# DaanVrancken/HubbardTN

Measured on AMD Instinct MI355X. Metric: DMRG sweep time (s) + GS energy/site, 1-band Hubbard L=64 chi=1024, lower is better.
Workload: dtype c128; 1 GPU; one-band Hubbard chain L=64 U/t=4, half filling, fZ2xSU(2)xU(1), two-site DMRG sweep (2L-3=125 bond updates) at chi=1024 (TensorKit dim units); model=one_band, L=64, chi=1024, krylovdim=30, parallelism=sector-parallel apply x1, backend=hip

## Files before the change

hubbardtn_amd/csrc/htn_svd.hip:

```cpp
#include <algorithm>
#include <utility>
#include <vector>

#include "htn_common.h"

#ifdef HTN_QR_PROF
#define QR_PROF 1
#else
#define QR_PROF 0
#endif
#ifdef HTN_RING_PROF
#define RING_PROF 1
#else
#define RING_PROF 0
#endif
#define JAC_T_1(var) const long long var = wall_clock64()
#define JAC_T_0(var)
#define JAC_ACC_1(arr, slot, a, b) arr[slot] += (b) - (a)
#define JAC_ACC_0(arr, slot, a, b)
#define JAC_PICK_(name, on) name##on
#define JAC_PICK(name, on) JAC_PICK_(name, on)
#define JAC_T(on, var) JAC_PICK(JAC_T_, on)(var)
#define JAC_ACC(on, arr, slot, a, b) JAC_PICK(JAC_ACC_, on)(arr, slot, a, b)

// ... 141 lines not shown
    static bool attr_set[64] = {};
    int dev = 0;
    HIP_TRY(hipGetDevice(&dev));
    std::lock_guard<std::mutex> lk(attr_mu);
    if (dev >= 0 && dev < 64 && !attr_set[dev]) {
        HIP_TRY(hipFuncSetAttribute((const void*)k_jacobi_svd, hipFuncAttributeMaxDynamicSharedMemorySize,
                                    JAC_LDS_ELEMS * (int)sizeof(double2)));
        HIP_TRY(hipFuncSetAttribute((const void*)k_qr_large, hipFuncAttributeMaxDynamicSharedMemorySize,
                                    16 * (64 * JAC_MAXEL + 1) * (int)sizeof(double2)));
        HIP_TRY(hipFuncSetAttribute((const void*)k_jacobi_pairs_gram, hipFuncAttributeMaxDynamicSharedMemorySize,
                                    (16 * (64 * JAC_MAXEL + 1) + JG_GU_ELEMS) * (int)sizeof(double2)));
        HIP_TRY(hipFuncSetAttribute((const void*)k_jacobi_ring, hipFuncAttributeMaxDynamicSharedMemorySize,
                                    2 * RING_PANEL_ELEMS * (int)sizeof(double2)));
        attr_set[dev] = true;
    }
    return 0;
}

static std::vector<int> classify_large(const htn_svd_block* desc_host, int n_blocks, int split) {
    const int large_min = split > 0 ? std::min(split, JAC_LDS_ELEMS) : JAC_LDS_ELEMS;
    std::vector<int> large;
    if (desc_host)
        for (int b = 0; b < n_blocks; ++b) {
            const htn_svd_block& D = desc_host[b];
            if (!(D.flags & HTN_SVD_QRCP) || D.n < 2) continue;
            if ((int64_t)jac_padded_rows(D.m) * D.n > large_min) large.push_back(b);
        }
    return large;
}

struct JacCoreBufs {
    int *d_ids, *d_slot, *d_perm;
    double* d_zero;
    unsigned long long* d_ratio;
    int *d_done, *d_sw;
    unsigned* d_qsync;
    JacPairItem* d_items;
    JacPairItem* h_items;
    int *h_ids, *h_slot;
    volatile int *h_active, *h_rank, *h_ring_sw;
    int *d_active, *d_rank, *d_ring_sw;
};
static int carve_core_scratch(JacScratch& js, int nl, int n_blocks, int max_sweeps, size_t n_items_max, JacCoreBufs* B) {
    const size_t off_ids = 0, off_slot = off_ids + sizeof(int) * nl, off_perm = off_slot + sizeof(int) * n_blocks;
    const size_t off_zero = off_perm + sizeof(int) * nl * 64 * JAC_MAXEL;
    const size_t off_ratio = (off_zero + sizeof(double) * nl + 7) / 8 * 8, off_done = off_ratio + 16 * nl;
    const size_t off_sw = off_done + sizeof(int) * nl, off_qsync = off_sw + sizeof(int) * nl;
    const size_t off_items = (off_qsync + sizeof(unsigned) * (QR_SYNC_WORDS * (size_t)nl + 8) + 31) / 32 * 32;
    if (js.dev.reserve(off_items + sizeof(JacPairItem) * n_items_max)) return 1;
    if (js.pinned.reserve(sizeof(JacPairItem) * n_items_max + 4 * (size_t)(nl + n_blocks) + 128)) return 1;
    if (js.flags.reserve(sizeof(int) * ((size_t)(max_sweeps + 1) + 2 * (size_t)nl + 16))) return 1;
    char* d = (char*)js.dev.p;
    B->d_ids = (int*)(d + off_ids);
    B->d_slot = (int*)(d + off_slot);
    B->d_perm = (int*)(d + off_perm);
    B->d_zero = (double*)(d + off_zero);
    B->d_ratio = (unsigned long long*)(d + off_ratio);
    B->d_done = (int*)(d + off_done);
    B->d_sw = (int*)(d + off_sw);
    B->d_qsync = (unsigned*)(d + off_qsync);
    B->d_items = (JacPairItem*)(d + off_items);
    char* h = (char*)js.pinned.p;
    B->h_items = (JacPairItem*)h;
    B->h_ids = (int*)(h + sizeof(JacPairItem) * n_items_max);
    B->h_slot = B->h_ids + nl;
    B->h_active = (volatile int*)js.flags.p;
    B->h_rank = B->h_active + (max_sweeps + 1);
    B->h_ring_sw = B->h_rank + nl;
    B->d_active = (int*)js.flags.dev;
    B->d_rank = B->d_active + (max_sweeps + 1);
    B->d_ring_sw = B->d_rank + nl;
    return 0;
}

struct RingPlan {
    std::vector<RingItem> items;
    std::vector<std::pair<int, int>> batches;
    int wgs = 0;
    int64_t mbox_elems = 0;
};
static bool plan_ring(const JacCall& c, int n_xcd, int ring_cap, RingPlan* plan) {
    *plan = RingPlan();
    struct Blk {
        int li, P, w, mp;
    };
    std::vector<Blk> blks;
    for (int li = 0; li < c.nl(); ++li) {
        const htn_svd_block& D = c.desc_host[c.large[li]];
        const int gsx = ring_gs(D.m);
        const int mp = gsx * ring_e(D.m);
        int wcap = std::min(RING_THREADS / gsx, RING_PANEL_ELEMS / mp);
        if (gsx == 16 && wcap > 16 && wcap < 32) wcap = 16;
        if (c.split > 0) wcap = std::min(wcap, 3);
        const int n = std::max(c.n_eff[li], 1);
        const int P = std::max(1, (n + 2 * wcap - 1) / (2 * wcap));
        if (wcap < 1 || P > RING_MAX_P || P > ring_cap) return false;
        blks.push_back({li, P, (n + 2 * P - 1) / (2 * P), mp});
    }
    std::stable_sort(blks.begin(), blks.end(), [](const Blk& a, const Blk& b) { return a.P > b.P; });
    std::vector<char> placed(blks.size(), 0);
    size_t left = blks.size();
    int nx = n_xcd;
    for (const Blk& B : blks)
        if (B.P > ring_cap / nx) nx = 1;
    const int lane_cap = ring_cap / nx;
    while (left) {
        const int first = (int)plan->items.size();
        std::vector<int> lane_used((size_t)nx, 0);
        struct Put {
            int q, x, s0;
        };
        std::vector<Put> puts;
        for (size_t q = 0; q < blks.size(); ++q) {
            if (placed[q]) continue;
            int x = 0;
            for (int y = 1; y < nx; ++y)
                if (lane_used[y] < lane_used[x]) x = y;
            if (lane_used[x] + blks[q].P > lane_cap) continue;
            puts.push_back({(int)q, x, lane_used[x]});
            lane_used[x] += blks[q].P;
            placed[q] = 1;
            --left;
        }
        int depth = 0;
        for (int y = 0; y < nx; ++y) depth = std::max(depth, lane_used[y]);
        const int grid = depth * nx;
        plan->items.resize((size_t)first + grid, RingItem{0, 0, 0, 0, 0, 0, 0});
        for (const Put& pt : puts) {
            const Blk& B = blks[pt.q];
            for (int k = 0; k < B.P; ++k)
                plan->items[(size_t)first + (size_t)(pt.s0 + k) * nx + pt.x] = {B.li, k, B.P, B.w, c.n_eff[B.li], plan->wgs,
                                                                                 plan->mbox_elems};
            plan->mbox_elems += (int64_t)B.P * 4 * B.w * B.mp;
            plan->wgs += B.P;
        }
        plan->batches.push_back({first, grid});
    }
    return true;
}

static int launch_qr_large(const JacCall& c, JacScratch& js, const JacCoreBufs& B, int n_xcd) {
    const int nl = c.nl();
    int max_m0 = 0, min_m0 = 1 << 30, max_n0 = 0;
    for (int b : c.large) {
        max_m0 = std::max(max_m0, (int)c.desc_host[b].pad);
        min_m0 = std::min(min_m0, (int)c.desc_host[b].pad);
        max_n0 = std::max(max_n0, (int)c.desc_host[b].m);
    }
    const size_t qr_panel_elems = (size_t)16 * (((max_m0 + 15) & ~15) + 1);
    const bool coop = ((min_m0 + 15) & ~15) <= 256 && qr_panel_elems * sizeof(double2) + 65536 + 30720 <= 163840;
    const size_t qr_lds = qr_panel_elems * sizeof(double2) + (coop ? 65536 : 0);
    static const bool qr_single = htn_env_flag("HTN_QR_SINGLE");
    static const int env_nw = getenv("HTN_QR_NW") ? atoi(getenv("HTN_QR_NW")) : 0;
    int NW = qr_single ? 1 : ((max_n0 >= 160 || js.xcd_local) ? 4 : 1);
    if (env_nw > 0 && !qr_single) NW = std::min(env_nw, 4);
    const int cus = std::max(1, std::min(js.cu_count > 0 ? js.cu_count : 256, 256));
    const int qnx = (NW > 1 && n_xcd > 1) ? n_xcd : 1;
    const int nl_pad = (nl + qnx - 1) / qnx * qnx;
    NW = std::max(1, std::min(NW, cus / std::max(nl_pad, 1)));
    if (NW > 1 && js.qr_box.reserve((size_t)nl * QR_BOX_BYTES)) return 1;
    const int qgrid_nx = NW > 1 ? qnx : 1;
    hipLaunchKernelGGL(k_qr_large, dim3((NW > 1 ? nl_pad : nl) * NW), dim3(JAC_THREADS), qr_lds, c.st, c.G, c.Vj, c.desc, B.d_ids,
                       B.d_perm, B.d_zero, c.cut2, B.d_rank, NW, (char*)js.qr_box.p, B.d_qsync, nl, qgrid_nx,
                       coop ? (int)qr_panel_elems : 0);
    return 0;
}

static int run_ring(const JacCall& c, JacScratch& js, const JacCoreBufs& B, const RingPlan& plan, int n_xcd, bool two_partner,
                    bool staged_send, int32_t* sweeps_used) {
    const int nl = c.nl(), n_wg = plan.wgs, n_items = (int)plan.items.size();
    const int arrive_off = 2 * n_wg, fail_off = arrive_off + nl * c.max_sweeps, xcc_off = fail_off + 1;
    const int conv_off = (xcc_off + n_wg + 3) & ~3;
    const size_t sync_bytes = ((size_t)conv_off * 4 + (size_t)nl * c.max_sweeps * 16 + 15) & ~(size_t)15;
    if (js.ring_sync.reserve(sync_bytes)) return 1;
    if (js.ring_mbox.reserve(sizeof(double2) * (size_t)std::max<int64_t>(plan.mbox_elems, 1))) return 1;
    if (js.ring_items.reserve(sizeof(RingItem) * n_items) || js.ring_items_h.reserve(sizeof(RingItem) * n_items)) return 1;
    memcpy(js.ring_items_h.p, plan.items.data(), sizeof(RingItem) * n_items);
    for (int li = 0; li < nl; ++li) B.h_ring_sw[li] = 0;
    HIP_TRY(hipMemcpyAsync(js.ring_items.p, js.ring_items_h.p, sizeof(RingItem) * n_items, hipMemcpyHostToDevice, c.st));
    HIP_TRY(hipMemsetAsync(js.ring_sync.p, 0, sync_bytes, c.st));
    RingArgs ra;
    ra.Vj = c.Vj, ra.G = c.G, ra.S = c.S, ra.desc = c.desc, ra.large_ids = B.d_ids;
    ra.perm = B.d_perm, ra.zero2 = B.d_zero, ra.mbox = (double2*)js.ring_mbox.p, ra.sync = (unsigned*)js.ring_sync.p;
    ra.arrive_off = arrive_off, ra.fail_off = fail_off, ra.conv_off = conv_off, ra.max_sweeps = c.max_sweeps, ra.tol = c.tol;
    ra.xcc_off = xcc_off;
    ra.two_partner = two_partner ? 1 : 0;
    ra.staged_send = staged_send ? 1 : 0;
    ra.info = c.info_dev, ra.sweeps_out = B.d_ring_sw;
    for (auto& bt : plan.batches) {
        ra.items = (const RingItem*)js.ring_items.p + bt.first;
        hipLaunchKernelGGL(k_jacobi_ring, dim3((unsigned)bt.second), dim3(RING_THREADS), 2 * RING_PANEL_ELEMS * sizeof(double2),
                           c.st, ra);
    }
    HIP_TRY(hipGetLastError());
    HIP_TRY(hipStreamWaitEvent(c.st, js.ev_join, 0));
    HIP_TRY(htn_stream_spin(c.st));
    int used = 0;
    for (int li = 0; li < nl; ++li) {
        if (B.h_rank[li] < 0) return fail_msg("htn_jacobi_svd_z: a hand-off of the multi-workgroup QR timed out");
        if (B.h_ring_sw[li] <= 0 && c.n_eff[li] >= 2)
            return fail_msg("htn_jacobi_svd_z: a hand-off of the ring Jacobi kernel timed out");
        used = std::max(used, (int)B.h_ring_sw[li] % 1000);
    }
    int all_local = n_xcd > 1 ? 1 : 0;
    for (int li = 0; li < nl; ++li)
        if (c.n_eff[li] >= 2 && B.h_ring_sw[li] < 1000) all_local = 0;
    js.xcd_local = all_local;
    if (sweeps_used) *sweeps_used = used;
    return 0;
}

static int run_pair_visits(const JacCall& c, JacScratch& js, const JacCoreBufs& B, const JacTournament& T, int hint,
                           int32_t* sweeps_used) {
    const int nl = c.nl();
    int max_mp = 0;
    for (int b : c.large) max_mp = std::max(max_mp, jac_padded_rows(c.desc_host[b].m));
    const size_t gram_lds_bytes = (size_t)(16 * (max_mp + 1) + JG_GU_ELEMS) * sizeof(double2);
    const int used = jacobi_sweep_pipeline(c.max_sweeps, hint, js.ev_sweep, B.h_active, c.st, [&](int sweep) {
        for (int r = 0; r < T.n_rounds(); ++r)
            if (T.round_size(r))
                hipLaunchKernelGGL(k_jacobi_pairs_gram, dim3(T.round_size(r)), dim3(256), gram_lds_bytes, c.st, c.Vj, c.desc,
                                   B.d_ids, B.d_items + T.off[r], B.d_zero, B.d_ratio, B.d_done, c.tol, 1);
        hipLaunchKernelGGL(k_jacobi_check, dim3(1), dim3(64), 0, c.st, B.d_ratio, B.d_done, B.d_sw, nl, c.tol, B.d_active + sweep);
    });
    if (used < 0) return 1;
    if (sweeps_used) *sweeps_used = used;
    HIP_TRY(hipStreamWaitEvent(c.st, js.ev_join, 0));
    hipLaunchKernelGGL(k_jacobi_finish, dim3(nl), dim3(JAC_THREADS), 0, c.st, c.G, (const double2*)c.Vj, c.S, c.desc, B.d_ids,
                       B.d_perm, B.d_sw, B.d_done, c.info_dev);
    HIP_TRY(hipGetLastError());
    HIP_TRY(htn_stream_spin(c.st));
    return 0;
}

static int jacobi_svd_core(void* G, void* Vj, double* S, const htn_svd_block* desc, const htn_svd_block* desc_host,
                           int32_t n_blocks, int32_t max_m_host, int32_t max_sweeps, double tol, int32_t* info_dev,
                           const htn_svd_opts* opts, void* stream, const int* skip_dev, const unsigned char* skip_host) {
    if (n_blocks <= 0) return 0;
    if (max_m_host > 64 * JAC_MAXEL) return fail_msg("htn_jacobi_svd_z: block taller than 512 rows");
    const double rank_cut = opts && opts->rank_cut > 0.0 ? opts->rank_cut : 0.0;
    JacCall c = {(double2*)G, (double2*)Vj, S, desc, desc_host, n_blocks, max_sweeps, tol, rank_cut * rank_cut,
                 opts && opts->split_elems > 0 ? opts->split_elems : 0, info_dev, (hipStream_t)stream, {}, {}};
    int32_t* sweeps_used = opts ? opts->sweeps_used : nullptr;
    if (jac_set_kernel_attributes()) return 1;
    c.large = classify_large(desc_host, n_blocks, c.split);
    if (sweeps_used) *sweeps_used = 0;
    if (c.large.empty()) {
        hipLaunchKernelGGL(k_jacobi_svd, dim3(n_blocks), dim3(JAC_THREADS), JAC_LDS_ELEMS * sizeof(double2), c.st, c.G, c.Vj, S,
                           desc, max_sweeps, tol, info_dev, JAC_LDS_ELEMS, skip_dev, c.cut2);
        HIP_TRY(hipGetLastError());
        return 0;
    }
    const int nl = c.nl();
    size_t n_items_max = 0;
    for (int b : c.large) {
        const int nb = (desc_host[b].n + JAC_PANEL - 1) / JAC_PANEL, nbp = nb + (nb & 1);
        n_items_max += (size_t)(nbp - 1) * (nbp / 2) + (nb + 1) / 2;
        c.n_eff.push_back(desc_host[b].n);
    }
    JacScratch* jsp = nullptr;
    JacCoreBufs B;
    if (js_get(c.st, &jsp) || carve_core_scratch(*jsp, nl, n_blocks, max_sweeps, n_items_max, &B)) return 1;
    JacScratch& js = *jsp;
    for (int b = 0; b < n_blocks; ++b) B.h_slot[b] = skip_host && skip_host[b] ? nl : -1;
    for (int li = 0; li < nl; ++li) B.h_slot[c.large[li]] = li;
    for (int li = 0; li < nl; ++li) B.h_ids[li] = c.large[li];
    for (int k = 0; k <= max_sweeps; ++k) B.h_active[k] = 1;
    HIP_TRY(hipMemcpyAsync(B.d_ids, B.h_ids, sizeof(int) * (nl + n_blocks), hipMemcpyHostToDevice, c.st));
    HIP_TRY(hipMemsetAsync(B.d_ratio, 0, 24 * (size_t)nl + sizeof(unsigned) * (QR_SYNC_WORDS * (size_t)nl + 8), c.st));
    static const bool force_pairs = htn_env_flag("HTN_SVD_PAIRS");
    static const bool no_xcd = htn_env_flag("HTN_RING_NO_XCD");
    static const bool ring_staged = htn_env_flag("HTN_RING_STAGED_SEND");
    const bool ring_two_partner = htn_env_flag("HTN_RING_TWO_PARTNER");
    const int n_xcd = (!no_xcd && js.cu_count > 0 && js.cu_count % 8 == 0) ? 8 : 1;
    const int ring_cap = std::max(1, std::min(js.cu_count > 0 ? js.cu_count : 256, 256));
    RingPlan plan;
    JacTournament T;
    bool use_ring = !force_pairs && plan_ring(c, n_xcd, ring_cap, &plan);
    if (c.cut2 <= 0.0 && !use_ring) {
        T = jacobi_tournament(c.n_eff.data(), nl);
        if (upload_tournament(T, B.h_items, B.d_items, c.st)) return 1;
    }
    HIP_TRY(hipEventRecord(js.ev_fork, c.st));
    HIP_TRY(hipStreamWaitEvent(js.aux, js.ev_fork, 0));
    hipLaunchKernelGGL(k_jacobi_svd, dim3(n_blocks), dim3(JAC_THREADS), JAC_LDS_ELEMS * sizeof(double2), js.aux, c.G, c.Vj, S,
                       desc, max_sweeps, tol, info_dev, JAC_LDS_ELEMS, (const int*)B.d_slot, c.cut2);
    HIP_TRY(hipEventRecord(js.ev_join, js.aux));
    if (launch_qr_large(c, js, B, n_xcd)) return 1;
    if (c.cut2 > 0.0) {
        HIP_TRY(hipEventRecord(js.ev_sweep[0], c.st));
        HIP_TRY(htn_event_spin(js.ev_sweep[0]));
        for (int li = 0; li < nl; ++li) c.n_eff[li] = std::min(c.n_eff[li], (int)B.h_rank[li]);
        if (use_ring) use_ring = plan_ring(c, n_xcd, ring_cap, &plan);
        if (!use_ring) {
            T = jacobi_tournament(c.n_eff.data(), nl);
            if (upload_tournament(T, B.h_items, B.d_items, c.st)) return 1;
        }
    }
    if (use_ring) return run_ring(c, js, B, plan, n_xcd, ring_two_partner, ring_staged, sweeps_used);
    return run_pair_visits(c, js, B, T, opts && opts->sweeps_hint > 0 ? opts->sweeps_hint : 0, sweeps_used);
}

static int jacobi_svd_tall(void* G, void* Vj, double* S, const htn_svd_block* desc, const htn_svd_block* desc_host,
                           int32_t n_blocks, int32_t max_m_rest, int32_t max_sweeps, double tol, int32_t* info_dev,
                           const htn_svd_opts* opts, void* stream, const std::vector<int>& tall) {
    const int nt = (int)tall.size();
    hipStream_t st = (hipStream_t)stream;
    JacScratch* jsp = nullptr;
    if (js_get(st, &jsp)) return 1;
    JacScratch& js = *jsp;
    std::vector<int> n_cols(nt);
    for (int li = 0; li < nt; ++li) n_cols[li] = desc_host[tall[li]].n;
// ... 86 lines not shown
```

hubbardtn_amd/csrc/htn_svd_qr.h:

```cpp
#pragma once

template <int GS>
__device__ __forceinline__ int qrcp_mgs(double2* __restrict__ g0, int m0, int n0, int r, const SplitCols X,
                                        int* s_col, double* s_cn2, double* s_piv, int tid, double cut2) {
    const int grp = tid / GS, sub = tid % GS, lane = tid & 63, wave = tid >> 6;
    const int ngroups = JAC_THREADS / GS;
    for (int idx = tid; idx < X.mp * r; idx += JAC_THREADS) X.col(idx / X.mp)[idx % X.mp] = make_double2(0.0, 0.0);
    for (int k = grp; k < n0; k += ngroups) {
        double c = 0.0;
        for (int i = sub; i < m0; i += GS) {
            const double2 x = g0[(int64_t)k * m0 + i];
            c += x.x * x.x + x.y * x.y;
        }
        c = group_sum<GS>(c);
        if (sub == 0) {
            s_cn2[k] = c;
            s_col[k] = k;
        }
    }
    __syncthreads();
    if (wave == 0) {
        double f = 0.0;
        for (int k = lane; k < n0; k += 64) f += s_cn2[k];
        f = wave_sum(f);
        if (lane == 0) s_piv[1] = 1e-30 * f;
    }
    __syncthreads();
    const double zero2 = s_piv[1];
    int rank = 0;
    for (int j = 0; j < r; ++j) {
        if (wave == 0) {
            double best = -1.0, mass = 0.0;
            int bi = j;
            for (int k = j + lane; k < n0; k += 64) {
                mass += s_cn2[k];
                if (s_cn2[k] > best) {
                    best = s_cn2[k];
                    bi = k;
                }
            }
            mass = wave_sum(mass);
#pragma unroll
            for (int off = 32; off > 0; off >>= 1) {
                const double ob = __shfl_xor(best, off, 64);
                const int oi = __shfl_xor(bi, off, 64);
                if (ob > best || (ob == best && oi < bi)) {
                    best = ob;
                    bi = oi;
                }
            }
            if (bi != j)
                for (int jj = lane; jj < j; jj += 64) {
                    double2* xc = X.col(jj);
                    const double2 t = xc[j];
                    xc[j] = xc[bi];
                    xc[bi] = t;
                }
            if (lane == 0) {
                const int t = s_col[j];
                s_col[j] = s_col[bi];
                s_col[bi] = t;
                s_cn2[bi] = s_cn2[j];
                s_cn2[j] = best;
                s_piv[0] = mass <= cut2 ? 0.0 : best;
            }
        }
        __syncthreads();
        if (s_piv[0] <= zero2) break;
        rank = j + 1;
        const double2* __restrict__ p = g0 + (int64_t)s_col[j] * m0;
        for (int k = j + grp; k < n0; k += ngroups) {
            double2 pv[JAC_MAXEL], av[JAC_MAXEL];
            double pp = 0.0, dr = 0.0, di = 0.0;
            double2* __restrict__ a = g0 + (int64_t)s_col[k] * m0;
#pragma unroll
            for (int e = 0; e < JAC_MAXEL; ++e) {
                const int i = sub + GS * e;
                if (i < m0) {
                    pv[e] = p[i];
                    pp += pv[e].x * pv[e].x + pv[e].y * pv[e].y;
                    if (k > j) {
                        av[e] = a[i];
                        dr += pv[e].x * av[e].x + pv[e].y * av[e].y;
                        di += pv[e].x * av[e].y - pv[e].y * av[e].x;
                    }
                }
            }
            pp = group_sum<GS>(pp);
            const double pn = sqrt(pp);
            if (k == j) {
                if (sub == 0) X.col(j)[j] = make_double2(pn, 0.0);
                continue;
            }
            dr = group_sum<GS>(dr);
            di = group_sum<GS>(di);
            const double fr = dr / pp, fi = di / pp;
            double c = 0.0;
#pragma unroll
            for (int e = 0; e < JAC_MAXEL; ++e) {
                const int i = sub + GS * e;
                if (i < m0) {
                    const double2 x = make_double2(av[e].x - (fr * pv[e].x - fi * pv[e].y),
                                                   av[e].y - (fr * pv[e].y + fi * pv[e].x));
                    a[i] = x;
                    c += x.x * x.x + x.y * x.y;
                }
            }
            c = group_sum<GS>(c);
            if (sub == 0) {
                s_cn2[k] = c;
                X.col(j)[k] = make_double2(dr / pn, -di / pn);
            }
        }
        __syncthreads();
    }
    __syncthreads();
    return rank;
}

__device__ __forceinline__ void lds_barrier() {
    asm volatile("s_waitcnt lgkmcnt(0)\n\ts_barrier" ::: "memory");
}

typedef unsigned int qr_u4 __attribute__((ext_vector_type(4)));
struct QrShare {
    int NW, role;
    bool local;
    double2* qn;
    int* scol;
    double* cn2;
    int* meta;
    unsigned* qflag;
    unsigned* hflag;
    unsigned* fail;
};
__device__ __forceinline__ bool qr_wait_ge(unsigned* flag, unsigned want, unsigned* fail) {
    const long long t0 = wall_clock64();
    for (unsigned spins = 1;; ++spins) {
        if (__hip_atomic_load(flag, __ATOMIC_RELAXED, __HIP_MEMORY_SCOPE_AGENT) >= want) return true;
        __builtin_amdgcn_s_sleep(1);
        if ((spins & 255u) == 0u) {
            if (__hip_atomic_load(fail, __ATOMIC_RELAXED, __HIP_MEMORY_SCOPE_AGENT) != 0u) return false;
            if (wall_clock64() - t0 > 300000000ll) {
                __hip_atomic_store(fail, 1u, __ATOMIC_RELAXED, __HIP_MEMORY_SCOPE_AGENT);
                return false;
            }
        }
    }
}
template <bool SH>
__device__ __forceinline__ double2 qr_ld(const double2* base, __amdgpu_buffer_rsrc_t rs, int idx) {
    if (!SH) return base[idx];
    const qr_u4 u = __builtin_amdgcn_raw_buffer_load_b128(rs, idx * 16, 0, 16);
    double2 v;
    __builtin_memcpy(&v, &u, 16);
    return v;
}
template <bool SH>
__device__ __forceinline__ void qr_st(double2* base, __amdgpu_buffer_rsrc_t rs, int idx, double2 v, bool local) {
    if (!SH) {
        base[idx] = v;
        return;
    }
    qr_u4 u;
    __builtin_memcpy(&u, &v, 16);
    if (local) __builtin_amdgcn_raw_buffer_store_b128(u, rs, idx * 16, 0, 0);
    else __builtin_amdgcn_raw_buffer_store_b128(u, rs, idx * 16, 0, 16);
}

template <bool SH>
__device__ __forceinline__ void qr_trailing_chunk(double2* __restrict__ g0, __amdgpu_buffer_rsrc_t rg, double2* __restrict__ Xg,
                                                  __amdgpu_buffer_rsrc_t rx, const double2* Qn, int ldq, const int* s_col, int m0,
                                                  int m0p, int n0, int mp, int j0, int nb_eff, int k_first, int ch, bool last_panel,
                                                  double* norm_out, bool norm_shared, int lane, bool local) {
    const int l15 = lane & 15, l4 = lane >> 4;
    const int nks = m0p >> 2;
    const int k = k_first + 16 * ch + l15;
    const bool valid = k < n0;
    const int pk = valid ? s_col[k] : 0;
    const int abase = pk * m0;
    d4 cr = {0.0, 0.0, 0.0, 0.0}, ci = {0.0, 0.0, 0.0, 0.0};
    const double2* qrow = Qn + l15 * ldq + l4;
    double2 ring[4];
#pragma unroll
    for (int u = 0; u < 4; ++u) {
        const int i = 4 * u + l4;
        ring[u] = (valid && u < nks && i < m0) ? qr_ld<SH>(g0, rg, abase + i) : make_double2(0.0, 0.0);
    }
    for (int ks0 = 0; ks0 < nks; ks0 += 4) {
#pragma unroll
        for (int u = 0; u < 4; ++u) {
            const int ks = ks0 + u;
            if (ks < nks) {
                const double2 b = ring[u];
                const int inx = 4 * (ks + 4) + l4;
                ring[u] = (valid && ks + 4 < nks && inx < m0) ? qr_ld<SH>(g0, rg, abase + inx) : make_double2(0.0, 0.0);
                const double2 qv = qrow[4 * ks];
                cr = __builtin_amdgcn_mfma_f64_16x16x4f64(qv.x, b.x, cr, 0, 0, 0);
                ci = __builtin_amdgcn_mfma_f64_16x16x4f64(qv.x, b.y, ci, 0, 0, 0);
                cr = __builtin_amdgcn_mfma_f64_16x16x4f64(qv.y, b.y, cr, 0, 0, 0);
                ci = __builtin_amdgcn_mfma_f64_16x16x4f64(-qv.y, b.x, ci, 0, 0, 0);
            }
        }
    }
#pragma unroll
    for (int reg = 0; reg < 4; ++reg) {
        const int t = l4 + 4 * reg;
        if (valid && t < nb_eff) qr_st<SH>(Xg, rx, (j0 + t) * mp + pk, make_double2(cr[reg], -ci[reg]), local);
    }
    if (last_panel) return;
    double nrm = 0.0;
    for (int i0 = 0; i0 < m0p; i0 += 16) {
        double2 old[4];
#pragma unroll
        for (int reg = 0; reg < 4; ++reg) {
            const int i = i0 + l4 + 4 * reg;
            old[reg] = (valid && i < m0) ? qr_ld<SH>(g0, rg, abase + i) : make_double2(0.0, 0.0);
        }
        d4 dr = {0.0, 0.0, 0.0, 0.0}, di = {0.0, 0.0, 0.0, 0.0};
#pragma unroll
        for (int kk = 0; kk < 4; ++kk) {
            const double2 qa = Qn[(l4 + 4 * kk) * ldq + i0 + l15];
            dr = __builtin_amdgcn_mfma_f64_16x16x4f64(qa.x, cr[kk], dr, 0, 0, 0);
            di = __builtin_amdgcn_mfma_f64_16x16x4f64(qa.x, ci[kk], di, 0, 0, 0);
            dr = __builtin_amdgcn_mfma_f64_16x16x4f64(-qa.y, ci[kk], dr, 0, 0, 0);
            di = __builtin_amdgcn_mfma_f64_16x16x4f64(qa.y, cr[kk], di, 0, 0, 0);
        }
#pragma unroll
        for (int reg = 0; reg < 4; ++reg) {
            const int i = i0 + l4 + 4 * reg;
            if (valid && i < m0) {
                const double2 x = make_double2(old[reg].x - dr[reg], old[reg].y - di[reg]);
                qr_st<SH>(g0, rg, abase + i, x, local);
                nrm += x.x * x.x + x.y * x.y;
            }
        }
    }
    nrm += __shfl_xor(nrm, 16, 64);
    nrm += __shfl_xor(nrm, 32, 64);
    if (valid && l4 == 0) {
        if (norm_shared) __hip_atomic_store(norm_out + k, nrm, __ATOMIC_RELAXED, __HIP_MEMORY_SCOPE_AGENT);
        else norm_out[k] = nrm;
    }
}

template <bool SH>
__device__ __forceinline__ void qr_trailing_coop(double2* __restrict__ g0, __amdgpu_buffer_rsrc_t rg, double2* __restrict__ Xg,
                                                 __amdgpu_buffer_rsrc_t rx, const double2* Qn, int ldq, const int* s_col, int m0,
                                                 int m0p, int n0, int mp, int j0, int nb_eff, int k_first, int nchunks, int role,
                                                 int NW, bool last_panel, double* norm_out, bool norm_shared, double* part,
                                                 int tid, bool local) {
    __shared__ double s_np[JAC_THREADS / 64][16];
    const int lane = tid & 63, wave = tid >> 6, l15 = lane & 15, l4 = lane >> 4;
    const int cnt = nchunks > role ? (nchunks - role + NW - 1) / NW : 0;
    if (part == nullptr) {
        for (int q = wave; q < cnt; q += JAC_THREADS / 64)
            qr_trailing_chunk<SH>(g0, rg, Xg, rx, Qn, ldq, s_col, m0, m0p, n0, mp, j0, nb_eff, k_first, role + NW * q, last_panel, norm_out,
                                  norm_shared, lane, local);
        return;
    }
    constexpr int S = 4, CPR = (JAC_THREADS / 64) / S;
    const int nks = m0p >> 2;
    for (int r0 = 0; r0 < cnt; r0 += CPR) {
        const int ci_ = r0 + wave / S, pp = wave % S;
        const bool act = ci_ < cnt;
        const int ch = role + NW * ci_;
        const int k = k_first + 16 * ch + l15;
        const bool valid = act && k < n0;
        const int pk = valid ? s_col[k] : 0;
        const int abase = pk * m0;
        d4 cr = {0.0, 0.0, 0.0, 0.0}, ci = {0.0, 0.0, 0.0, 0.0};
        if (act) {
            const double2* qrow = Qn + l15 * ldq + l4;
            double2 ring[4];
#pragma unroll
            for (int u = 0; u < 4; ++u) {
                const int ks = 4 * pp + u, i = 4 * ks + l4;
                ring[u] = (valid && ks < nks && i < m0) ? qr_ld<SH>(g0, rg, abase + i) : make_double2(0.0, 0.0);
            }
            for (int ks0 = 4 * pp; ks0 < nks; ks0 += 4 * S) {
#pragma unroll
                for (int u = 0; u < 4; ++u) {
                    const int ks = ks0 + u;
                    if (ks < nks) {
                        const double2 b = ring[u];
                        const int ksn = ks + 4 * S, inx = 4 * ksn + l4;
                        ring[u] = (valid && ksn < nks && inx < m0) ? qr_ld<SH>(g0, rg, abase + inx) : make_double2(0.0, 0.0);
                        const double2 qv = qrow[4 * ks];
                        cr = __builtin_amdgcn_mfma_f64_16x16x4f64(qv.x, b.x, cr, 0, 0, 0);
                        ci = __builtin_amdgcn_mfma_f64_16x16x4f64(qv.x, b.y, ci, 0, 0, 0);
                        cr = __builtin_amdgcn_mfma_f64_16x16x4f64(qv.y, b.y, cr, 0, 0, 0);
                        ci = __builtin_amdgcn_mfma_f64_16x16x4f64(-qv.y, b.x, ci, 0, 0, 0);
                    }
                }
            }
        }
        {
            double* mine = part + (size_t)wave * 512 + lane;
#pragma unroll
            for (int reg = 0; reg < 4; ++reg) {
                mine[64 * reg] = cr[reg];
                mine[64 * (4 + reg)] = ci[reg];
            }
        }
        __syncthreads();
        {
            const double* base = part + (size_t)(wave - pp) * 512 + lane;
#pragma unroll
            for (int reg = 0; reg < 4; ++reg) {
                double a = 0.0, b = 0.0;
#pragma unroll
                for (int q = 0; q < S; ++q) {
                    a += base[q * 512 + 64 * reg];
                    b += base[q * 512 + 64 * (4 + reg)];
                }
                cr[reg] = a;
                ci[reg] = b;
            }
        }
        if (pp == 0) {
#pragma unroll
            for (int reg = 0; reg < 4; ++reg) {
                const int t = l4 + 4 * reg;
                if (valid && t < nb_eff) qr_st<SH>(Xg, rx, (j0 + t) * mp + pk, make_double2(cr[reg], -ci[reg]), local);
            }
        }
        if (!last_panel) {
            double nrm = 0.0;
            if (act) {
                for (int i0 = 16 * pp; i0 < m0p; i0 += 16 * S) {
                    double2 old[4];
#pragma unroll
                    for (int reg = 0; reg < 4; ++reg) {
                        const int i = i0 + l4 + 4 * reg;
                        old[reg] = (valid && i < m0) ? qr_ld<SH>(g0, rg, abase + i) : make_double2(0.0, 0.0);
                    }
                    d4 dr = {0.0, 0.0, 0.0, 0.0}, di = {0.0, 0.0, 0.0, 0.0};
#pragma unroll
                    for (int kk = 0; kk < 4; ++kk) {
                        const double2 qa = Qn[(l4 + 4 * kk) * ldq + i0 + l15];
                        dr = __builtin_amdgcn_mfma_f64_16x16x4f64(qa.x, cr[kk], dr, 0, 0, 0);
                        di = __builtin_amdgcn_mfma_f64_16x16x4f64(qa.x, ci[kk], di, 0, 0, 0);
                        dr = __builtin_amdgcn_mfma_f64_16x16x4f64(-qa.y, ci[kk], dr, 0, 0, 0);
                        di = __builtin_amdgcn_mfma_f64_16x16x4f64(qa.y, cr[kk], di, 0, 0, 0);
                    }
#pragma unroll
                    for (int reg = 0; reg < 4; ++reg) {
                        const int i = i0 + l4 + 4 * reg;
                        if (valid && i < m0) {
                            const double2 x = make_double2(old[reg].x - dr[reg], old[reg].y - di[reg]);
                            qr_st<SH>(g0, rg, abase + i, x, local);
                            nrm += x.x * x.x + x.y * x.y;
                        }
                    }
                }
            }
            nrm += __shfl_xor(nrm, 16, 64);
            nrm += __shfl_xor(nrm, 32, 64);
            if (l4 == 0) s_np[wave][l15] = nrm;
            __syncthreads();
            if (valid && pp == 0 && l4 == 0) {
                double t = 0.0;
#pragma unroll
                for (int q = 0; q < S; ++q) t += s_np[wave + q][l15];
                if (norm_shared) __hip_atomic_store(norm_out + k, t, __ATOMIC_RELAXED, __HIP_MEMORY_SCOPE_AGENT);
                else norm_out[k] = t;
            }
        }
        __syncthreads();
    }
}

__device__ __forceinline__ void qr_helper(double2* __restrict__ g0, int m0, int n0, int r, double2* __restrict__ Xg, int mp, int* s_col,
                                          double2* Qn, int tid, const QrShare sh, double* part) {
    __shared__ int s_meta[8];
    const int lane = tid & 63, wave = tid >> 6;
    const int m0p = (m0 + 15) & ~15, ldq = m0p + 1;
    const __amdgpu_buffer_rsrc_t rg = __builtin_amdgcn_make_buffer_rsrc((void*)g0, 0, m0 * n0 * 16, 0x00020000);
    const __amdgpu_buffer_rsrc_t rx = __builtin_amdgcn_make_buffer_rsrc((void*)Xg, 0, mp * r * 16, 0x00020000);
    const __amdgpu_buffer_rsrc_t rq = __builtin_amdgcn_make_buffer_rsrc((void*)sh.qn, 0, 16 * ldq * 16, 0x00020000);
    for (unsigned epoch = 1;; ++epoch) {
        if (tid == 0) {
            const bool ok = qr_wait_ge(sh.qflag, epoch, sh.fail);
            s_meta[5] = ok ? 0 : 1;
            for (int q = 0; q < 5; ++q) s_meta[q] = ok ? __hip_atomic_load(sh.meta + q, __ATOMIC_RELAXED, __HIP_MEMORY_SCOPE_AGENT) : 0;
        }
        __syncthreads();
        const int j0 = s_meta[0], nb_eff = s_meta[1], k_first = s_meta[2];
        const bool last_panel = s_meta[3] != 0, finished = s_meta[4] != 0 || s_meta[5] != 0;
        if (finished) break;
        for (int idx = tid; idx < 16 * ldq; idx += JAC_THREADS) Qn[idx] = qr_ld<true>(sh.qn, rq, idx);
        for (int k = k_first + tid; k < n0; k += JAC_THREADS) s_col[k] = __hip_atomic_load(sh.scol + k, __ATOMIC_RELAXED, __HIP_MEMORY_SCOPE_AGENT);
        __syncthreads();
        const int nchunks = (n0 - k_first + 15) >> 4;
        qr_trailing_coop<true>(g0, rg, Xg, rx, Qn, ldq, s_col, m0, m0p, n0, mp, j0, nb_eff, k_first, nchunks, sh.role, sh.NW, last_panel, sh.cn2,
                               true, part, tid, sh.local);
        asm volatile("s_waitcnt vmcnt(0)" ::: "memory");
        __syncthreads();
        if (tid == 0) __hip_atomic_store(sh.hflag + sh.role, epoch, __ATOMIC_RELAXED, __HIP_MEMORY_SCOPE_AGENT);
    }
}

#ifdef HTN_QR_PROF
__device__ long long g_qr_prof[8];
extern "C" int htn_qr_prof_dump(long long* out) {
    HIP_TRY(hipDeviceSynchronize());
    HIP_TRY(hipMemcpyFromSymbol(out, HIP_SYMBOL(g_qr_prof), sizeof(long long) * 8));
    return 0;
}
#endif
template <int EL, bool SH>
__device__ __forceinline__ int qrcp_blocked(double2* __restrict__ g0, int m0, int n0, int r,
                                            double2* __restrict__ Xg, int mp, int* s_col, double* s_cn2,
                                            double* s_piv, double2* Qn, int tid, double cut2, const QrShare sh, double* part) {
    __shared__ double s_pn[16];
    __shared__ int s_share_ok;
    const __amdgpu_buffer_rsrc_t rg = __builtin_amdgcn_make_buffer_rsrc((void*)g0, 0, m0 * n0 * 16, 0x00020000);
    const __amdgpu_buffer_rsrc_t rx = __builtin_amdgcn_make_buffer_rsrc((void*)Xg, 0, mp * r * 16, 0x00020000);
    unsigned pub_epoch = 0;
    if (tid == 0) s_share_ok = 1;
    __shared__ double2 s_r[16][17];
    __shared__ int s_pc[16];
    __shared__ int s_pos[16];
    __shared__ int s_nb;
    const int lane = tid & 63, wave = tid >> 6, l15 = lane & 15, l4 = lane >> 4;
    const int m0p = (m0 + 15) & ~15, ldq = m0p + 1;
    for (int idx = tid; idx < mp * r; idx += JAC_THREADS) qr_st<SH>(Xg, rx, idx, make_double2(0.0, 0.0), sh.local);
    for (int k = wave; k < n0; k += JAC_THREADS / 64) {
        double c = 0.0;
        for (int i = lane; i < m0; i += 64) {
            const double2 x = g0[(int64_t)k * m0 + i];
            c += x.x * x.x + x.y * x.y;
        }
        c = wave_sum(c);
        if (lane == 0) {
            s_cn2[k] = c;
            s_col[k] = k;
        }
    }
    __syncthreads();
    if (wave == 0) {
        double f = 0.0;
        for (int k = lane; k < n0; k += 64) f += s_cn2[k];
        f = wave_sum(f);
        if (lane == 0) s_piv[1] = 1e-30 * f;
    }
    __syncthreads();
    const double zero2 = s_piv[1];
    bool stop = false;
    int j0 = 0, rank = 0;
#ifdef HTN_QR_PROF
    long long qprof[8] = {0, 0, 0, 0, 0, 0, 0, 0};
    const long long qt0 = wall_clock64();
#endif
    while (j0 < r && !stop) {
        JAC_T(QR_PROF, q0);
        const int nbmax = r - j0 < 16 ? r - j0 : 16;
        if (wave == 0) {
            int nb = 0;
            double mass = 0.0;
            for (int k = j0 + lane; k < n0; k += 64) mass += s_cn2[k];
            mass = wave_sum(mass);
            for (int t = 0; t < (mass <= cut2 ? 0 : nbmax); ++t) {
                const int j = j0 + t;
                unsigned long long key = 0ull;
                for (int k = j + lane; k < n0; k += 64) {
                    const unsigned long long kk =
                        ((unsigned long long)__double_as_longlong(s_cn2[k]) & ~0x3FFull) | (unsigned long long)(1023 - k);
                    key = kk > key ? kk : key;
                }
                key = wave_max_u64(key);
                const int bi = 1023 - (int)(key & 0x3FFull);
                const double best = s_cn2[bi];
                if (best <= zero2) break;
                if (lane == 0) {
                    const int tc = s_col[j];
                    s_col[j] = s_col[bi];
                    s_col[bi] = tc;
                    s_cn2[bi] = s_cn2[j];
                    s_cn2[j] = best;
                }
                ++nb;
            }
            if (lane == 0) s_nb = nb;
        }
        __syncthreads();
        JAC_T(QR_PROF, q1);
        JAC_ACC(QR_PROF, qprof, 0, q0, q1);
        int nb = s_nb;
        if (nb == 0) break;
        if (nb < nbmax) stop = true;
        const bool owner = wave < nb;
        const int pc = owner ? s_col[j0 + wave] : 0;
        double2 a[EL];
        double cn = owner ? s_cn2[j0 + wave] : -1.0;
        const double ns = cn;
#pragma unroll
        for (int e = 0; e < EL; ++e) {
            const int i = lane + 64 * e;
            a[e] = (owner && i < m0) ? qr_ld<SH>(g0, rg, pc * m0 + i) : make_double2(0.0, 0.0);
        }
        if (!owner)
            for (int i = lane; i < m0p; i += 64) Qn[wave * ldq + i] = make_double2(0.0, 0.0);
        if (tid < 256) s_r[tid >> 4][tid & 15] = make_double2(0.0, 0.0);
        if (lane == 0) s_pc[wave] = pc;
        bool pending = owner;
        int nb_eff = nb;
        JAC_T(QR_PROF, q2);
        JAC_ACC(QR_PROF, qprof, 1, q1, q2);
        for (int t = 0; t < nb; ++t) {
            if (lane == 0) s_pn[wave] = pending ? cn : -1.0;
            lds_barrier();
            unsigned long long key = 0ull;
            {
                const double v = s_pn[l15];
                if (v >= 0.0) key = ((unsigned long long)__double_as_longlong(v) & ~0xFull) | (unsigned long long)(15 - l15);
            }
            key = row_max16_u64(key);
            const int bu = 15 - (int)(key & 0xFull);
            const double best = key ? s_pn[bu] : -1.0;
            if (best <= zero2) {
                nb_eff = t;
                stop = true;
                break;
            }
            if (wave == bu) {
                if (cn < 1e-4 * ns) {
                    for (int s2 = 0; s2 < t; ++s2) {
                        double dr = 0.0, di = 0.0;
                        const double2* qs = Qn + s2 * ldq + lane;
#pragma unroll
                        for (int e = 0; e < EL; ++e) {
                            if (lane + 64 * e < m0p) {
                                const double2 q = qs[64 * e];
                                dr += q.x * a[e].x + q.y * a[e].y;
                                di += q.x * a[e].y - q.y * a[e].x;
                            }
                        }
                        dr = wave_sum(dr);
                        di = wave_sum(di);
#pragma unroll
                        for (int e = 0; e < EL; ++e) {
                            if (lane + 64 * e < m0p) {
                                const double2 q = qs[64 * e];
                                a[e].x -= dr * q.x - di * q.y;
                                a[e].y -= dr * q.y + di * q.x;
                            }
                        }
                        if (lane == 0) {
                            const double2 old = s_r[s2][wave];
                            s_r[s2][wave] = make_double2(old.x + dr, old.y - di);
                        }
                    }
                    double c = 0.0;
#pragma unroll
                    for (int e = 0; e < EL; ++e) c += a[e].x * a[e].x + a[e].y * a[e].y;
                    cn = wave_sum(c);
                }
                const double ipn = fast_rsq(cn);
                const double pn = cn * ipn;
#pragma unroll
                for (int e = 0; e < EL; ++e) {
                    const int i = lane + 64 * e;
                    if (i < m0p) Qn[t * ldq + i] = make_double2(a[e].x * ipn, a[e].y * ipn);
                }
                if (lane == 0) {
                    s_r[t][wave] = make_double2(pn, 0.0);
                    s_pos[t] = pc;
                }
                pending = false;
            }
            lds_barrier();
            if (pending) {
                double dr = 0.0, di = 0.0;
                const double2* qt = Qn + t * ldq + lane;
#pragma unroll
                for (int e = 0; e < EL; ++e) {
                    if (lane + 64 * e < m0p) {
                        const double2 q = qt[64 * e];
                        dr += q.x * a[e].x + q.y * a[e].y;
                        di += q.x * a[e].y - q.y * a[e].x;
                    }
                }
                dr = wave_sum(dr);
                di = wave_sum(di);
                double c = 0.0;
#pragma unroll
                for (int e = 0; e < EL; ++e) {
                    if (lane + 64 * e < m0p) {
                        const double2 q = qt[64 * e];
                        a[e].x -= dr * q.x - di * q.y;
                        a[e].y -= dr * q.y + di * q.x;
                        c += a[e].x * a[e].x + a[e].y * a[e].y;
                    }
                }
                cn = wave_sum(c);
                if (lane == 0) s_r[t][wave] = make_double2(dr, -di);
            }
        }
        __syncthreads();
        JAC_T(QR_PROF, q3);
        JAC_ACC(QR_PROF, qprof, 2, q2, q3);
        if (nb_eff < nb) {
            for (int tt = nb_eff + wave; tt < nb; tt += JAC_THREADS / 64)
                for (int i = lane; i < m0p; i += 64) Qn[tt * ldq + i] = make_double2(0.0, 0.0);
        }
        if (tid < nb_eff) s_col[j0 + tid] = s_pos[tid];
        if (tid < 256 && (tid >> 4) < nb_eff && (tid & 15) < nb)
            qr_st<SH>(Xg, rx, (j0 + (tid >> 4)) * mp + s_pc[tid & 15], s_r[tid >> 4][tid & 15], sh.local);
        __syncthreads();
        JAC_T(QR_PROF, q4);
        JAC_ACC(QR_PROF, qprof, 3, q3, q4);
        const int k_first = j0 + nb;
        const int nchunks = (n0 - k_first + 15) >> 4;
        const bool last_panel = stop || k_first >= r;
        const int NW = SH ? sh.NW : 1;
        if (SH && nchunks > 0) {
            const __amdgpu_buffer_rsrc_t rq = __builtin_amdgcn_make_buffer_rsrc((void*)sh.qn, 0, 16 * ldq * 16, 0x00020000);
            for (int idx = tid; idx < 16 * ldq; idx += JAC_THREADS) qr_st<true>(sh.qn, rq, idx, Qn[idx], sh.local);
            for (int k = k_first + tid; k < n0; k += JAC_THREADS) __hip_atomic_store(sh.scol + k, s_col[k], __ATOMIC_RELAXED, __HIP_MEMORY_SCOPE_AGENT);
            if (tid == 0) {
                __hip_atomic_store(sh.meta + 0, j0, __ATOMIC_RELAXED, __HIP_MEMORY_SCOPE_AGENT);
                __hip_atomic_store(sh.meta + 1, nb_eff, __ATOMIC_RELAXED, __HIP_MEMORY_SCOPE_AGENT);
                __hip_atomic_store(sh.meta + 2, k_first, __ATOMIC_RELAXED, __HIP_MEMORY_SCOPE_AGENT);
                __hip_atomic_store(sh.meta + 3, last_panel ? 1 : 0, __ATOMIC_RELAXED, __HIP_MEMORY_SCOPE_AGENT);
                __hip_atomic_store(sh.meta + 4, 0, __ATOMIC_RELAXED, __HIP_MEMORY_SCOPE_AGENT);
            }
            asm volatile("s_waitcnt vmcnt(0)" ::: "memory");
            __syncthreads();
            ++pub_epoch;
            if (tid == 0) __hip_atomic_store(sh.qflag, pub_epoch, __ATOMIC_RELAXED, __HIP_MEMORY_SCOPE_AGENT);
        }
        qr_trailing_coop<SH>(g0, rg, Xg, rx, Qn, ldq, s_col, m0, m0p, n0, mp, j0, nb_eff, k_first, nchunks, 0, NW, last_panel, s_cn2, false, part,
                             tid, sh.local);
        if (SH && nchunks > 0) {
            asm volatile("s_waitcnt vmcnt(0)" ::: "memory");
            __syncthreads();
            if (tid == 0) {
                bool ok = true;
                for (int h = 1; h < NW && ok; ++h) ok = qr_wait_ge(sh.hflag + h, pub_epoch, sh.fail);
                if (!ok) s_share_ok = 0;
            }
            __syncthreads();
            if (!s_share_ok) {
                stop = true;
            } else if (!last_panel) {
                for (int k = k_first + tid; k < n0; k += JAC_THREADS)
                    if (((k - k_first) >> 4) % NW != 0) s_cn2[k] = __hip_atomic_load(sh.cn2 + k, __ATOMIC_RELAXED, __HIP_MEMORY_SCOPE_AGENT);
            }
        }
        __syncthreads();
        JAC_T(QR_PROF, q5);
        JAC_ACC(QR_PROF, qprof, 4, q4, q5);
#ifdef HTN_QR_PROF
        qprof[6] += 1;
#endif
        j0 += nb;
        rank += nb_eff;
    }
    __syncthreads();
#ifdef HTN_QR_PROF
    if (tid == 0 && blockIdx.x == 0) {
        qprof[5] = wall_clock64() - qt0;
        for (int q = 0; q < 8; ++q) g_qr_prof[q] = qprof[q];
    }
#endif
    if (SH) {
        if (tid == 0) {
            __hip_atomic_store(sh.meta + 4, 1, __ATOMIC_RELAXED, __HIP_MEMORY_SCOPE_AGENT);
            asm volatile("s_waitcnt vmcnt(0)" ::: "memory");
            __hip_atomic_store(sh.qflag, pub_epoch + 1, __ATOMIC_RELAXED, __HIP_MEMORY_SCOPE_AGENT);
        }
        __syncthreads();
        if (!s_share_ok) rank = -1;
    }
    for (int i = tid; i < n0; i += JAC_THREADS) s_col[i] = i;
    __syncthreads();
    return rank;
}

#define QR_SYNC_WORDS 16
#define QR_BOX_BYTES 137728
__global__ __launch_bounds__(JAC_THREADS) void k_qr_large(double2* __restrict__ G, double2* __restrict__ Vj,
                                                          const htn_svd_block* __restrict__ desc,
                                                          const int* __restrict__ large_ids, int* __restrict__ perm,
                                                          double* __restrict__ zero2_out, double cut2,
                                                          int* __restrict__ rank_host, int NW, char* __restrict__ qr_box,
                                                          unsigned* __restrict__ qr_sync, int nl, int nx, int part_off) {
    extern __shared__ double2 g_lds[];
    __shared__ double s_piv[2];
    __shared__ int s_col[64 * JAC_MAXEL];
    __shared__ double s_cn2[64 * JAC_MAXEL];
    __shared__ int s_qlocal;
    const int px = (int)(blockIdx.x % (unsigned)nx), ps = (int)(blockIdx.x / (unsigned)nx);
    const int li = (ps / NW) * nx + px, role = ps % NW;
    if (li >= nl) return;
    const htn_svd_block D = desc[large_ids[li]];
    const int m = D.m, n = D.n, m0 = D.pad, tid = threadIdx.x;
    const int gsx = m <= 16 * JAC_MAXEL ? 16 : (m <= 32 * JAC_MAXEL ? 32 : 64);
    const int mp = gsx * ((m + gsx - 1) / gsx);
    double2* __restrict__ X = Vj + D.v_off;
    QrShare sh;
    sh.NW = NW, sh.role = role;
    char* box = qr_box + (size_t)li * QR_BOX_BYTES;
    sh.qn = (double2*)box;
    sh.scol = (int*)(box + 16 * 513 * 16);
    sh.cn2 = (double*)(box + 16 * 513 * 16 + 512 * 4);
    sh.meta = (int*)(box + 16 * 513 * 16 + 512 * 4 + 512 * 8);
    sh.qflag = qr_sync + li * QR_SYNC_WORDS;
    sh.hflag = qr_sync + li * QR_SYNC_WORDS + 1;
    sh.fail = qr_sync + nl * QR_SYNC_WORDS;
    sh.local = false;
    if (NW > 1) {
        if (tid == 0) {
            unsigned xcc;
            asm volatile("s_getreg_b32 %0, hwreg(HW_REG_XCC_ID)" : "=s"(xcc));
            xcc = (xcc & 0xfu) + 1u;
            unsigned* xw = qr_sync + li * QR_SYNC_WORDS + 8;
            __hip_atomic_store(xw + role, xcc, __ATOMIC_RELAXED, __HIP_MEMORY_SCOPE_AGENT);
            int local = 1;
            for (int q = 0; q < NW && local >= 0; ++q) {
                if (!qr_wait_ge(xw + q, 1u, sh.fail)) local = -1;
                else if (__hip_atomic_load(xw + q, __ATOMIC_RELAXED, __HIP_MEMORY_SCOPE_AGENT) != xcc) local = 0;
            }
            s_qlocal = local;
        }
        __syncthreads();
        sh.local = s_qlocal > 0;
    }
    double* part = (part_off > 0 && ((m0 + 15) & ~15) <= 256) ? (double*)(g_lds + part_off) : nullptr;
    if (role > 0) {
        qr_helper(G + D.g_off, m0, m, n, X, mp, s_col, (double2*)g_lds, tid, sh, part);
        return;
    }
    int rank;
    if (NW > 1) {
        if (m0 <= 256) rank = qrcp_blocked<4, true>(G + D.g_off, m0, m, n, X, mp, s_col, s_cn2, s_piv, (double2*)g_lds, tid, cut2, sh, part);
        else rank = qrcp_blocked<8, true>(G + D.g_off, m0, m, n, X, mp, s_col, s_cn2, s_piv, (double2*)g_lds, tid, cut2, sh, part);
    } else {
        if (m0 <= 256) rank = qrcp_blocked<4, false>(G + D.g_off, m0, m, n, X, mp, s_col, s_cn2, s_piv, (double2*)g_lds, tid, cut2, sh, part);
        else rank = qrcp_blocked<8, false>(G + D.g_off, m0, m, n, X, mp, s_col, s_cn2, s_piv, (double2*)g_lds, tid, cut2, sh, part);
    }
    if (tid == 0) {
        rank_host[li] = rank;
        zero2_out[li] = s_piv[1];
        __threadfence_system();
    }
    for (int i = tid; i < m; i += JAC_THREADS) perm[li * 64 * JAC_MAXEL + i] = s_col[i];
}
```

Measured before the change: 397.2 ms.

## Scale QR helper workgroups with column chunks and use wave-parallel flag waits

The number of cooperating workgroups per large QR block now scales with the number of 16-column chunks, capped at 16 instead of a fixed 4. It is also limited by the CUs available per XCD. Helper waits on the per-helper and XCC flags now use one lane per flag with a wave vote, replacing a serial loop on thread 0. Helpers with no chunk in the current panel skip loading Q and the trailing update. The intent is more parallelism in the trailing QR update. In exchange there is more synchronization traffic per panel, a larger sync-word layout, and a risk of CU oversubscription.

```diff
diff --git a/hubbardtn_amd/csrc/htn_svd.hip b/hubbardtn_amd/csrc/htn_svd.hip
--- a/hubbardtn_amd/csrc/htn_svd.hip
+++ b/hubbardtn_amd/csrc/htn_svd.hip
@@ -317,12 +317,14 @@
     const size_t qr_lds = qr_panel_elems * sizeof(double2) + (coop ? 65536 : 0);
     static const bool qr_single = htn_env_flag("HTN_QR_SINGLE");
     static const int env_nw = getenv("HTN_QR_NW") ? atoi(getenv("HTN_QR_NW")) : 0;
-    int NW = qr_single ? 1 : ((max_n0 >= 160 || js.xcd_local) ? 4 : 1);
-    if (env_nw > 0 && !qr_single) NW = std::min(env_nw, 4);
+    const int chunks = std::max(1, (max_n0 - 16 + 15) / 16);
+    int NW = qr_single ? 1 : ((max_n0 >= 160 || js.xcd_local) ? std::min(chunks, QR_NW_CAP) : 1);
+    if (env_nw > 0 && !qr_single) NW = std::min(env_nw, QR_MAX_NW);
     const int cus = std::max(1, std::min(js.cu_count > 0 ? js.cu_count : 256, 256));
     const int qnx = (NW > 1 && n_xcd > 1) ? n_xcd : 1;
     const int nl_pad = (nl + qnx - 1) / qnx * qnx;
     NW = std::max(1, std::min(NW, cus / std::max(nl_pad, 1)));
+    if (qnx > 1) NW = std::max(1, std::min(NW, (cus / qnx) / (nl_pad / qnx)));
     if (NW > 1 && js.qr_box.reserve((size_t)nl * QR_BOX_BYTES)) return 1;
     const int qgrid_nx = NW > 1 ? qnx : 1;
     hipLaunchKernelGGL(k_qr_large, dim3((NW > 1 ? nl_pad : nl) * NW), dim3(JAC_THREADS), qr_lds, c.st, c.G, c.Vj, c.desc, B.d_ids,
diff --git a/hubbardtn_amd/csrc/htn_svd_qr.h b/hubbardtn_amd/csrc/htn_svd_qr.h
--- a/hubbardtn_amd/csrc/htn_svd_qr.h
+++ b/hubbardtn_amd/csrc/htn_svd_qr.h
@@ -148,6 +148,26 @@
         }
     }
 }
+__device__ __forceinline__ bool qr_wait_lanes_ge(unsigned* words, int lo, int hi, unsigned want, unsigned* fail, int lane, unsigned* got) {
+    const bool mine = lane >= lo && lane < hi;
+    const long long t0 = wall_clock64();
+    unsigned v = want;
+    for (unsigned spins = 1;; ++spins) {
+        if (mine) v = __hip_atomic_load(words + lane, __ATOMIC_RELAXED, __HIP_MEMORY_SCOPE_AGENT);
+        if (__all(v >= want)) {
+            *got = v;
+            return true;
+        }
+        __builtin_amdgcn_s_sleep(1);
+        if ((spins & 255u) == 0u) {
+            if (__hip_atomic_load(fail, __ATOMIC_RELAXED, __HIP_MEMORY_SCOPE_AGENT) != 0u) return false;
+            if (wall_clock64() - t0 > 300000000ll) {
+                if (lane == 0) __hip_atomic_store(fail, 1u, __ATOMIC_RELAXED, __HIP_MEMORY_SCOPE_AGENT);
+                return false;
+            }
+        }
+    }
+}
 template <bool SH>
 __device__ __forceinline__ double2 qr_ld(const double2* base, __amdgpu_buffer_rsrc_t rs, int idx) {
     if (!SH) return base[idx];
@@ -389,13 +409,15 @@
         const int j0 = s_meta[0], nb_eff = s_meta[1], k_first = s_meta[2];
         const bool last_panel = s_meta[3] != 0, finished = s_meta[4] != 0 || s_meta[5] != 0;
         if (finished) break;
-        for (int idx = tid; idx < 16 * ldq; idx += JAC_THREADS) Qn[idx] = qr_ld<true>(sh.qn, rq, idx);
-        for (int k = k_first + tid; k < n0; k += JAC_THREADS) s_col[k] = __hip_atomic_load(sh.scol + k, __ATOMIC_RELAXED, __HIP_MEMORY_SCOPE_AGENT);
-        __syncthreads();
         const int nchunks = (n0 - k_first + 15) >> 4;
-        qr_trailing_coop<true>(g0, rg, Xg, rx, Qn, ldq, s_col, m0, m0p, n0, mp, j0, nb_eff, k_first, nchunks, sh.role, sh.NW, last_panel, sh.cn2,
-                               true, part, tid, sh.local);
-        asm volatile("s_waitcnt vmcnt(0)" ::: "memory");
+        if (nchunks > sh.role) {
+            for (int idx = tid; idx < 16 * ldq; idx += JAC_THREADS) Qn[idx] = qr_ld<true>(sh.qn, rq, idx);
+            for (int k = k_first + tid; k < n0; k += JAC_THREADS) s_col[k] = __hip_atomic_load(sh.scol + k, __ATOMIC_RELAXED, __HIP_MEMORY_SCOPE_AGENT);
+            __syncthreads();
+            qr_trailing_coop<true>(g0, rg, Xg, rx, Qn, ldq, s_col, m0, m0p, n0, mp, j0, nb_eff, k_first, nchunks, sh.role, sh.NW, last_panel,
+                                   sh.cn2, true, part, tid, sh.local);
+            asm volatile("s_waitcnt vmcnt(0)" ::: "memory");
+        }
         __syncthreads();
         if (tid == 0) __hip_atomic_store(sh.hflag + sh.role, epoch, __ATOMIC_RELAXED, __HIP_MEMORY_SCOPE_AGENT);
     }
@@ -636,10 +658,10 @@
         if (SH && nchunks > 0) {
             asm volatile("s_waitcnt vmcnt(0)" ::: "memory");
             __syncthreads();
-            if (tid == 0) {
-                bool ok = true;
-                for (int h = 1; h < NW && ok; ++h) ok = qr_wait_ge(sh.hflag + h, pub_epoch, sh.fail);
-                if (!ok) s_share_ok = 0;
+            if (wave == 0) {
+                unsigned got;
+                const bool ok = qr_wait_lanes_ge(sh.hflag, 1, NW, pub_epoch, sh.fail, lane, &got);
+                if (!ok && lane == 0) s_share_ok = 0;
             }
             __syncthreads();
             if (!s_share_ok) {
@@ -679,7 +701,9 @@
     return rank;
 }
 
-#define QR_SYNC_WORDS 16
+#define QR_MAX_NW 32
+#define QR_NW_CAP 16
+#define QR_SYNC_WORDS 64
 #define QR_BOX_BYTES 137728
 __global__ __launch_bounds__(JAC_THREADS) void k_qr_large(double2* __restrict__ G, double2* __restrict__ Vj,
                                                           const htn_svd_block* __restrict__ desc,
@@ -708,22 +732,21 @@
     sh.cn2 = (double*)(box + 16 * 513 * 16 + 512 * 4);
     sh.meta = (int*)(box + 16 * 513 * 16 + 512 * 4 + 512 * 8);
     sh.qflag = qr_sync + li * QR_SYNC_WORDS;
-    sh.hflag = qr_sync + li * QR_SYNC_WORDS + 1;
+    sh.hflag = qr_sync + li * QR_SYNC_WORDS;
     sh.fail = qr_sync + nl * QR_SYNC_WORDS;
     sh.local = false;
     if (NW > 1) {
-        if (tid == 0) {
+        if (tid < 64) {
             unsigned xcc;
             asm volatile("s_getreg_b32 %0, hwreg(HW_REG_XCC_ID)" : "=s"(xcc));
             xcc = (xcc & 0xfu) + 1u;
-            unsigned* xw = qr_sync + li * QR_SYNC_WORDS + 8;
-            __hip_atomic_store(xw + role, xcc, __ATOMIC_RELAXED, __HIP_MEMORY_SCOPE_AGENT);
-            int local = 1;
-            for (int q = 0; q < NW && local >= 0; ++q) {
-                if (!qr_wait_ge(xw + q, 1u, sh.fail)) local = -1;
-                else if (__hip_atomic_load(xw + q, __ATOMIC_RELAXED, __HIP_MEMORY_SCOPE_AGENT) != xcc) local = 0;
-            }
-            s_qlocal = local;
+            unsigned* xw = qr_sync + li * QR_SYNC_WORDS + QR_MAX_NW;
+            if (tid == 0) __hip_atomic_store(xw + role, xcc, __ATOMIC_RELAXED, __HIP_MEMORY_SCOPE_AGENT);
+            unsigned got = 0u;
+            const bool ok = qr_wait_lanes_ge(xw, 0, NW, 1u, sh.fail, tid, &got);
+            const bool same = tid >= NW || got == xcc;
+            const int local = !ok ? -1 : (__all(same) ? 1 : 0);
+            if (tid == 0) s_qlocal = local;
         }
         __syncthreads();
         sh.local = s_qlocal > 0;
```

Result: no change. 395.6 ms (median of 2 runs) (-0.4%).
